# lingo-db/lingo-db

Hardware: AMD Instinct MI355X
Metric: tpch_sf100_geomean_ms (lower is better)
Workload: dtype int64/int128 decimal

## Files before the change

lingo-db_amd/csrc/ldb_core.hip:

```cpp
#include "ldb_internal.h"
#include "ldb_device.h"
#include "ldb_chain.h"
#include <algorithm>
#include <cstdlib>
#include <memory>

static thread_local char g_err[1024] = "";
void ldb_set_error(const char* fmt, ...) {
   va_list ap;
   va_start(ap, fmt);
   vsnprintf(g_err, sizeof(g_err), fmt, ap);
   va_end(ap);
}
extern "C" const char* ldb_gpu_last_error(void) { return g_err; }

#include <atomic>
#include <functional>
#include <mutex>
static std::mutex g_opt_mu;
static std::atomic<int64_t> g_option_epoch{0};
static std::unordered_map<std::string, int64_t> g_opts;
int64_t ldb_option(const char* name, int64_t dflt) {
   std::lock_guard<std::mutex> lock(g_opt_mu);
   auto it = g_opts.find(name);
   if (it != g_opts.end()) return it->second;
   std::string env = "LDB_";
   for (const char* c = name; *c; c++) env += (char) toupper((unsigned char) *c);
   int64_t v = dflt;
   if (const char* e = getenv(env.c_str())) v = atoll(e);
   g_opts[name] = v;
   return v;
}
extern "C" int32_t ldb_gpu_set_option(const char* name, int64_t value) {
   if (!name) LDB_FAIL(LDB_ERR_INVALID, "set_option: NULL name");
   static const char* known[] = {"jit", "jit_min_rows", "lazy_filter", "lazy_min_rows", "join_ordered", "join_chained", "gb_ordered", "gb_sorted", "zone_maps", "zone_min_rows", "gb_direct", "gb_wgs_per_cu", "gb_partition", "gb_partition_min_rows", "join_radix", "join_radix_min_rows", "join_radix_min_table_bytes", "join_radix_part_bytes", "probe_batch", "debug_check", "join_direct", "join_rank", "join_coarse", "dict_encode", "dict_min_rows", "comm_transport", "comm_timeout_ms", "desc_cache", "desc_cache_mb", "plan_replay", "scan_single_pass", "lazy_strings", "lazy_strings_min_rows", "gb_partition_wc", "join_radix_wc", "join_radix_lds", "gb_dense_out", "gb_partition_values", "join_pair32", "gb_dense_keys", "jit_async", "jit_threads", "jit_disk_cache", "join_all_match", "topk_short_select", "gb_fits64", "join_coarse_fine", "join_coarse_filtered", "compact_wide_tiles", "compact_max_words", "join_fuse_max_conjuncts", "join_coarse_finest", "jit_min_rows_like", "scan_split", "jit_share_compiles"};
   bool ok = false;
   for (const char* k : known) ok |= strcmp(k, name) == 0;
   if (!ok) LDB_FAIL(LDB_ERR_INVALID, "set_option: unknown option '%s'", name);
   std::lock_guard<std::mutex> lock(g_opt_mu);
   g_opts[name] = value;
   g_option_epoch.fetch_add(1);
   return LDB_OK;
}
extern "C" int64_t ldb_gpu_get_option(const char* name) {
   if (!name) return -1;
   std::lock_guard<std::mutex> lock(g_opt_mu);
   auto it = g_opts.find(name);
   if (it != g_opts.end()) return it->second;
   std::string env = "LDB_";
   for (const char* c = name; *c; c++) env += (char) toupper((unsigned char) *c);
   if (const char* e = getenv(env.c_str())) return atoll(e);
   return -1;
}

double ldb_host_trace_threshold() {
   static const double thr = [] {
      const char* e = getenv("LDB_HOST_TRACE");
      return e && *e ? atof(e) : -1.0;
   }();
   return thr;
}
static size_t ldb_size_class(size_t bytes) {
   if (bytes <= 256) return 256;
   const int lg = 63 - __builtin_clzll((unsigned long long) (bytes - 1));
   const size_t step = (size_t) 1 << (lg >= 3 ? lg - 3 : 0);
   return (bytes + step - 1) / step * step;
}
static void ldb_cache_release(ldb_ctx* ctx) {
   for (auto& kv : ctx->parked)
      for (void* p : kv.second) (void) hipFreeAsync(p, ctx->stream);
   ctx->parked.clear();
   ctx->cache_bytes = 0;
}
int32_t ldb_dev_alloc(ldb_ctx* ctx, void** out, size_t bytes) {
   const size_t cls = ctx->cache_on ? ldb_size_class(bytes + 16) : bytes + 16;
   if (ctx->cache_on) {
      auto it = ctx->parked.find(cls);
      if (it != ctx->parked.end() && !it->second.empty()) {
         std::pop_heap(it->second.begin(), it->second.end(), std::greater<void*>());
         *out = it->second.back();
         it->second.pop_back();
         ctx->cache_bytes -= cls;
         ctx->live[*out] = cls;
         return LDB_OK;
      }
   }
   hipError_t e;
   {
      LdbSlow slow_("hipMallocAsync", cls);
      e = hipMallocAsync(out, cls, ctx->stream);
   }
   if (e != hipSuccess && ctx->cache_bytes) {
      (void) hipGetLastError();
      ldb_cache_release(ctx);
      (void) hipStreamSynchronize(ctx->stream);
      e = hipMallocAsync(out, cls, ctx->stream);
   }
   LDB_HIP(e);
   if (ctx->cache_on) ctx->live[*out] = cls;
   return LDB_OK;
}
void ldb_dev_free(ldb_ctx* ctx, void* p) {
   if (!p) return;
   auto dref = ctx->desc_blocks.find(p);
   if (dref != ctx->desc_blocks.end()) {
      if (dref->second > 0) dref->second--;
      else {
         ctx->desc_underflows++;
         if (ldb_host_trace_threshold() >= 0) fprintf(stderr, "[ldb] descriptor %p given back twice\n", p);
      }
      return;
   }
   if (!ctx->shared.empty()) {
      auto sh = ctx->shared.find(p);
      if (sh != ctx->shared.end()) {
         if (--sh->second == 0) ctx->shared.erase(sh);
         return;
      }
// ... 2030 lines not shown
```

lingo-db_amd/csrc/ldb_join.hip:

```cpp
#include "ldb_internal.h"
#include "ldb_join_kernel.h"
#include "ldb_jit.h"
#include <cmath>
#include "ldb_chain.h"
#include <algorithm>
#include <memory>

struct ldb_hashtable {
   ldb_ctx* ctx = nullptr;
   ldb_rel* build = nullptr;
   std::vector<ldb_colref> keys;
   uint64_t* slots = nullptr;
   uint64_t cap = 0;
   int32_t key32 = 0;
   int32_t unique = 0;
   int32_t ordered_slots = 0;
   int64_t kmin = 0, kmax = -1;
   uint64_t kmult = 0;
   uint32_t kmult32 = 0, ksh = 0;
   int32_t slot32 = 0;
   uint32_t* key_bits = nullptr;
   int32_t chained = 0;
   uint32_t* next = nullptr;
   int32_t direct = 0;
// ... 12 lines not shown
   }
};

__global__ void k_join_build(const DJoin* __restrict__ d);
__global__ void k_join_key_range(const DJoin* __restrict__ d, long long* __restrict__ out);
__global__ void k_join_key_bits(const DJoin* __restrict__ d);
__global__ void k_join_rank_bits(const DJoin* __restrict__ d);
__global__ void k_join_rank_perm(const DJoin* __restrict__ d);
__global__ void k_rank_coarse(const uint64_t* __restrict__ tab, uint64_t n_words, uint32_t* __restrict__ coarse, uint32_t coarse_words, uint32_t shift) {
   for (uint32_t c = blockIdx.x * blockDim.x + threadIdx.x; c < coarse_words; c += gridDim.x * blockDim.x) {
      uint32_t m = 0;
      for (uint32_t b = 0; b < 32; b++) {
         const uint64_t bit = (uint64_t) c * 32 + b;
         uint32_t any;
         if (shift == 6) {
            const uint64_t w = bit * 2;
            any = (w < n_words ? (uint32_t) tab[w] : 0u) | (w + 1 < n_words ? (uint32_t) tab[w + 1] : 0u);
         } else if (shift == 5) {
            any = bit < n_words ? (uint32_t) tab[bit] : 0u;
         } else {
            const uint64_t w = bit >> (5u - shift);
            const uint32_t piece = (uint32_t) (bit & ((1u << (5u - shift)) - 1u)), width = 1u << shift;
            any = w < n_words ? ((uint32_t) tab[w] >> (piece * width)) & ((1u << width) - 1u) : 0u;
         }
         if (any) m |= 1u << b;
      }
      coarse[c] = m;
   }
}
__global__ __launch_bounds__(256) void k_rank_prefix_chain(uint64_t* __restrict__ tab, uint64_t n_words, uint64_t n_tiles, unsigned long long* __restrict__ total,
                                                           unsigned long long* __restrict__ status, unsigned long long* __restrict__ ticket, unsigned long long ticket_base,
                                                           unsigned long long epoch) {
   __shared__ unsigned long long s_tile;
   __shared__ uint32_t s_wave[4];
   __shared__ uint32_t s_prefix;
   if (threadIdx.x == 0) s_tile = atomicAdd(ticket, 1ull) - ticket_base;
   __syncthreads();
   const uint64_t tile = s_tile;
   const uint64_t base = tile * CHAIN_TILE + (uint64_t) threadIdx.x * CHAIN_ITEMS;
   uint32_t bits[CHAIN_ITEMS];
   uint32_t sum = 0;
#pragma unroll
   for (int k = 0; k < CHAIN_ITEMS; k++) {
      bits[k] = base + k < n_words ? (uint32_t) tab[base + k] : 0u;
      sum += (uint32_t) __popc(bits[k]);
   }
   uint32_t agg;
   uint32_t excl = d_block_scan256<uint32_t>(sum, s_wave, &agg);
   if (threadIdx.x < 64) {
      const uint32_t prefix = d_chain_prefix<uint32_t, 32>(status, tile, epoch, agg, threadIdx.x);
      if (threadIdx.x == 0) s_prefix = prefix;
   }
   __syncthreads();
   excl += s_prefix;
   if (total && tile == n_tiles - 1 && threadIdx.x == 0) *total = (unsigned long long) s_prefix + agg;
#pragma unroll
   for (int k = 0; k < CHAIN_ITEMS; k++) {
      if (base + k < n_words) tab[base + k] = (uint64_t) bits[k] | ((uint64_t) excl << 32);
      excl += (uint32_t) __popc(bits[k]);
   }
}
__global__ void k_join_probe_pairs(const DJoin* __restrict__ d);
__global__ void k_join_probe_pairs_count(const DJoin* __restrict__ d);
__global__ void k_join_probe_count(const DJoin* __restrict__ d);
__global__ void k_join_probe_exists(const DJoin* __restrict__ d);
__global__ void k_join_probe_unique(const DJoin* __restrict__ d);
__global__ void k_join_probe_markbuild(const DJoin* __restrict__ d);
__global__ void k_join_flags_bitmap(const uint8_t* __restrict__ flags, uint64_t n, int anti, uint64_t* __restrict__ bitmap, unsigned long long* __restrict__ counter) {
   join_flags_bitmap_body(flags, n, anti, bitmap, counter);
}
__global__ void k_join_flags_bitmap2(const uint8_t* __restrict__ flags, const uint8_t* __restrict__ not_flags, uint64_t n, uint64_t* __restrict__ bitmap, unsigned long long* __restrict__ counter) {
   join_flags_bitmap_body(flags, n, 0, bitmap, counter, not_flags);
}

static const char* JOIN_SPEC_SRC =
   "extern \"C\" __global__ void k_join_build_spec(const DJoin* __restrict__ d) { join_build_body(LDB_META, d); }\n"
   "extern \"C\" __global__ void k_join_probe_pairs_spec(const DJoin* __restrict__ d) { join_probe_pairs_body(LDB_META, d); }\n"
   "extern \"C\" __global__ void k_join_probe_pairs_count_spec(const DJoin* __restrict__ d) { join_probe_pairs_count_body(LDB_META, d); }\n"
   "extern \"C\" __global__ void k_join_probe_count_spec(const DJoin* __restrict__ d) { join_probe_count_body(LDB_META, d); }\n"
   "extern \"C\" __global__ void k_join_probe_exists_spec(const DJoin* __restrict__ d) { join_probe_exists_body(LDB_META, d); }\n"
   "extern \"C\" __global__ void k_join_probe_unique_spec(const DJoin* __restrict__ d) { join_probe_unique_body(LDB_META, d); }\n"
   "extern \"C\" __global__ void k_join_probe_markbuild_spec(const DJoin* __restrict__ d) { join_probe_markbuild_body(LDB_META, d); }\n";

typedef void (*join_kernel_t)(const DJoin*);
static int32_t launch_join(ldb_ctx* ctx, const DJoin* h, const DJoin* d, int grid, const char* prof_name, const char* spec_name, join_kernel_t generic) {
   hipFunction_t spec = nullptr;
   if (ldb_jit_wanted((int64_t) h->n_rows)) {
      auto meta = std::make_unique<DJoin>();
      memcpy(meta.get(), h, sizeof(DJoin));
      meta->n_rows = meta->cap = meta->slots = meta->out_probe = meta->out_build = meta->out_cap = 0;
      meta->counter = meta->bitmap = meta->mark = meta->mark2 = meta->match = meta->flags = 0;
      meta->kmin = meta->kmax = 0;
      meta->kmult = 0;
      meta->kmult32 = meta->ksh = 0;
      meta->key_bits = 0;
      meta->next = 0;
      meta->coarse = 0;
      meta->coarse_words = 0;
      ldb_jit_strip_keys(meta->bkeys);
      ldb_jit_strip_keys(meta->pkeys);
      for (int p = 0; p < LDB_MAX_PREDS; p++) ldb_jit_strip_pred(meta->ppreds[p]);
      for (int p = 0; p < LDB_MAX_M2PREDS; p++) ldb_jit_strip_pred(meta->m2preds[p]);
      for (int k = 0; k < LDB_MAX_RESID; k++) {
         ldb_jit_strip_col(meta->resid[k].pcol);
         ldb_jit_strip_col(meta->resid[k].bcol);
      }
      std::string why;
      std::string one;
      for (const char* line = JOIN_SPEC_SRC; *line;) {
         const char* nl = strchr(line, '\n');
         const size_t len = nl ? (size_t) (nl - line) + 1 : strlen(line);
         std::string l(line, len);
         if (l.find(std::string(" ") + spec_name + "(") != std::string::npos) one = l;
         line += len;
      }
      spec = ldb_jit_kernel(ctx->device, "ldb_join_kernel.h", "DJoin", one.empty() ? JOIN_SPEC_SRC : one.c_str(), spec_name, meta.get(), sizeof(DJoin), &why);
   }
   const unsigned lds = h->has_coarse ? 4u * h->coarse_words : 0u;
   const bool big_lds = lds > 40u * 1024u;
   const bool tiles = h->n_ppreds > 0;
   const unsigned block = (h->has_coarse && !tiles) ? (big_lds ? 1024u : 512u) : 256u;
   if (h->has_coarse && !tiles) grid = (int) std::max<int64_t>(1, std::min<int64_t>(((int64_t) h->n_rows + block - 1) / block, (int64_t) ctx->cus * (big_lds ? 1 : 4)));
   if (big_lds) {
      if (spec) (void) hipFuncSetAttribute((const void*) spec, hipFuncAttributeMaxDynamicSharedMemorySize, (int) lds);
      else (void) hipFuncSetAttribute((const void*) generic, hipFuncAttributeMaxDynamicSharedMemorySize, (int) lds);
      (void) hipGetLastError();
   }
   LdbProf prof_(ctx, prof_name);
   if (spec) {
      void* params[] = {(void*) &d};
      LDB_HIP(hipModuleLaunchKernel(spec, (unsigned) grid, 1, 1, block, 1, 1, lds, ctx->stream, params, nullptr));
   } else {
      hipLaunchKernelGGL(generic, dim3(grid), dim3(block), lds, ctx->stream, d);
   }
   LDB_HIP(hipGetLastError());
   return LDB_OK;
}

bool ldb_join_jit_check(std::string* log) {
   auto m = std::make_unique<DJoin>();
   memset(m.get(), 0, sizeof(DJoin));
   m->key32 = 1;
   m->kind = LDB_JOIN_INNER;
   m->has_bitmap = 1;
   m->ordered_slots = 1;
   m->has_key_bits = 1;
   m->build_unique = 1;
   m->slot32 = 1;
   m->bkeys.n_keys = m->pkeys.n_keys = 1;
   m->bkeys.cols[0].type = m->pkeys.cols[0].type = LDB_T_INT32;
   m->bkeys.cols[0].width = m->pkeys.cols[0].width = 4;
   m->n_ppreds = 2;
   for (int p = 0; p < 2; p++) {
      m->ppreds[p].col.type = LDB_T_DATE32;
      m->ppreds[p].col.width = 4;
      m->ppreds[p].op = p ? LDB_F_LTE : LDB_F_GTE;
      m->ppreds[p].lo = p ? 9861 : 9131;
      m->ppreds[p].same_col = p;
   }
   if (const char* shape = getenv("LDB_JIT_CHECK_SHAPE")) {
      if (!strcmp(shape, "fk_count")) {
         m->n_ppreds = 0;
         m->has_key_bits = 0;
         m->has_bitmap = 0;
      }
   }
   if (!ldb_jit_compile_only("ldb_join_kernel.h", "DJoin", JOIN_SPEC_SRC, m.get(), sizeof(DJoin), log)) return false;
   m->n_ppreds = 0;
   m->ordered_slots = 0;
   m->slot32 = 0;
   m->has_key_bits = 0;
   m->direct = 1;
   if (!ldb_jit_compile_only("ldb_join_kernel.h", "DJoin", JOIN_SPEC_SRC, m.get(), sizeof(DJoin), log)) return false;
   m->direct = 2;
   m->rank_sorted = 1;
   if (!ldb_jit_compile_only("ldb_join_kernel.h", "DJoin", JOIN_SPEC_SRC, m.get(), sizeof(DJoin), log)) return false;
   m->rank_sorted = 0;
   m->kind = LDB_JOIN_SEMI;
   if (!ldb_jit_compile_only("ldb_join_kernel.h", "DJoin", JOIN_SPEC_SRC, m.get(), sizeof(DJoin), log)) return false;
   m->rank_sorted = 1;
   m->has_coarse = 32 | 6;
   return ldb_jit_compile_only("ldb_join_kernel.h", "DJoin", JOIN_SPEC_SRC, m.get(), sizeof(DJoin), log);
}

__global__ void k_word_pop(const uint64_t* __restrict__ bitmap, uint32_t* __restrict__ pop, uint64_t n_words) {
   for (uint64_t w = blockIdx.x * (uint64_t) blockDim.x + threadIdx.x; w < n_words; w += (uint64_t) gridDim.x * blockDim.x) pop[w] = (uint32_t) __popcll(bitmap[w]);
}
__global__ void k_bitmap_expand(const uint64_t* __restrict__ bitmap, const uint32_t* __restrict__ word_off, uint32_t* __restrict__ out, uint64_t n_words) {
   const uint32_t lane = threadIdx.x & 63;
   const uint64_t wave = (blockIdx.x * (uint64_t) blockDim.x + threadIdx.x) >> 6;
   const uint64_t n_waves = ((uint64_t) gridDim.x * blockDim.x) >> 6;
   for (uint64_t w = wave; w < n_words; w += n_waves) {
      uint64_t m = bitmap[w];
      if ((m >> lane) & 1) out[word_off[w] + d_rank_in(m)] = (uint32_t) (w * 64 + lane);
   }
}
__global__ void k_bitmap_expand_sparse(const uint64_t* __restrict__ bitmap, const uint32_t* __restrict__ word_off, uint32_t* __restrict__ out, uint64_t n_words) {
   for (uint64_t w = blockIdx.x * (uint64_t) blockDim.x + threadIdx.x; w < n_words; w += (uint64_t) gridDim.x * blockDim.x) {
      uint64_t m = bitmap[w];
      if (!m) continue;
      uint32_t at = word_off[w];
      const uint32_t base = (uint32_t) (w * 64);
      while (m) {
         out[at++] = base + (uint32_t) __builtin_ctzll(m);
         m &= m - 1;
// ... 330 lines not shown
   ht->unique = build_unique;
   auto hp = std::make_unique<DJoin>();
   DJoin* h = hp.get();
   memset(h, 0, sizeof(*h));
   LDB_TRY(ldb_make_dkeys(build, keys, n_keys, &h->bkeys));
   const DCol& k0 = h->bkeys.cols[0];
   ht->key32 = (n_keys == 1 && (k0.type == LDB_T_INT32 || k0.type == LDB_T_DATE32 || k0.type == LDB_T_CHAR4 || k0.type == LDB_T_INT16 || k0.type == LDB_T_INT8)) ? 1 : 0;
   ht->cap = std::max<uint64_t>(64, next_pow2_u64((uint64_t) build->n_rows * 2));
   h->n_rows = (uint64_t) build->n_rows;
   h->key32 = ht->key32;
   uint32_t* dflags;
   LDB_TRY(ldb_counters(ctx, 1, (uint64_t**) &dflags));
   h->flags = (uint64_t) dflags;
   h->has_flags = 1;
   const bool ordered_enabled = ldb_option("join_ordered", 1) != 0;
   if (ht->key32 && ordered_enabled && build->n_rows > 0) {
      long long got[2];
      const ldb_table* kt = build->sides[(size_t) keys[0].side].table;
      int64_t clo = 0, chi = -1;
      if (!kt->cols[(size_t) keys[0].col].validity && ldb_column_range(ctx, kt, keys[0].col, &clo, &chi) == LDB_OK && clo <= chi) {
         got[0] = clo;
         got[1] = chi;
      } else {
         long long* range = (long long*) (ctx->d_scratch + 32);
         const long long init[2] = {INT64_MAX, INT64_MIN};
         LDB_TRY(ldb_h2d_small(ctx, range, init, 16));
         LdbDesc<DJoin> dr_desc(ctx);
         LDB_TRY(dr_desc.upload(h, sizeof(*h)));
         DJoin* dr = dr_desc.p;
         hipLaunchKernelGGL(k_join_key_range, dim3(ldb_grid_for(ctx, build->n_rows, 256, 8)), dim3(256), 0, ctx->stream, dr, range);
         LDB_TRY(LDB_READBACK(ctx, got, range, 16));
         dr_desc.release();
      }
      const unsigned __int128 range0 = got[0] <= got[1] ? (unsigned __int128) ((__int128) got[1] - got[0]) + 1 : 0;
      bool ranked = false;
      if (range0 > 0 && build_unique && ldb_option("join_direct", 1) != 0 && ldb_option("join_rank", 1) != 0 && range0 <= ((unsigned __int128) 1 << 32) &&
          (range0 <= (unsigned __int128) std::max<int64_t>(4096, 64 * build->n_rows) || range0 <= ((unsigned __int128) 1 << 26)) && got[0] >= INT32_MIN && got[1] <= INT32_MAX && build->n_rows < (int64_t) LDB_NULL_ROW) {
         const uint64_t n_words = (uint64_t) (range0 / 32) + 1;
         uint64_t* tab = nullptr;
         LDB_TRY(ldb_dev_alloc(ctx, (void**) &tab, 8 * (size_t) n_words));
         ht->slots = tab;
         LDB_HIP(hipMemsetAsync(tab, 0, 8 * (size_t) n_words, ctx->stream));
         unsigned long long* counter;
         LDB_TRY(ldb_counters(ctx, 3, (uint64_t**) &counter));
         uint64_t* d_total = (uint64_t*) (counter + 2);
         h->direct = 2;
         h->kmin = got[0];
         h->kmax = got[1];
         h->slots = (uint64_t) tab;
         h->counter = (uint64_t) counter;
         LdbDesc<DJoin> dr_desc(ctx);
         LDB_TRY(dr_desc.upload(h, sizeof(*h)));
         DJoin* dr = dr_desc.p;
         {
            LdbProf prof_(ctx, "k_join_build");
            hipLaunchKernelGGL(k_join_rank_bits, dim3(ldb_grid_for(ctx, build->n_rows, 256, 8)), dim3(256), 0, ctx->stream, dr);
            const uint64_t n_tiles = (n_words + CHAIN_TILE - 1) / CHAIN_TILE;
            ChainCall c;
            LDB_TRY(ldb_chain_begin(ctx, n_tiles, false, &c));
            hipLaunchKernelGGL(k_rank_prefix_chain, dim3((unsigned) n_tiles), dim3(256), 0, ctx->stream, tab, n_words, n_tiles, (unsigned long long*) d_total, c.status, c.ticket, c.ticket_base, c.epoch);
            if (hipGetLastError() != hipSuccess) return ldb_chain_failed(ctx);
         }
         uint64_t back[3] = {0, 0, 0};
         uint32_t fl[2] = {0, 0};
         LDB_TRY(LDB_READBACK(ctx, back, counter, 24));
         LDB_TRY(LDB_READBACK(ctx, fl, dflags, 8));
         if (back[0] == back[2]) {
            ranked = true;
            ht->direct = 2;
            ht->kmin = got[0];
            ht->kmax = got[1];
            ht->cap = (uint64_t) range0;
            ht->slot_bytes = 8 * (size_t) n_words;
            ht->rank_sorted = (fl[0] & 4u) ? 0 : 1;
            uint32_t shift = 6;
            uint64_t cwords = (uint64_t) (range0 / 64 / 32) + 1;
            const double density = range0 > 0 ? (double) back[2] / (double) range0 : 1.0;
            const double pass64 = 1.0 - pow(1.0 - density, 64.0), pass16 = 1.0 - pow(1.0 - density, 16.0);
            const bool coarse_on = ldb_option("join_coarse", 1) != 0;
            bool want = coarse_on && cwords * 4 <= 40 * 1024 && (unsigned __int128) back[2] * 64 * 2 <= range0;
            if (coarse_on && ldb_option("join_coarse_fine", 1) != 0 && pass16 <= 0.7) {
               const uint64_t fine_words = (uint64_t) (range0 / 16 / 32) + 1;
               const bool small = fine_words * 4 <= 40 * 1024;
               if (small || (fine_words * 4 <= 156 * 1024 && (!want || pass64 > 0.25))) {
                  shift = 4;
                  cwords = fine_words;
                  want = true;
               }
            }
            if (coarse_on && ldb_option("join_coarse_finest", 1) != 0 && want && shift == 4 && cwords * 4 <= 16 * 1024) {
               while (shift > 0 && ((uint64_t) (range0 >> (shift - 1)) / 32 + 1) * 4 <= 16 * 1024 && 1.0 - pow(1.0 - density, (double) (1u << shift)) > 0.1) shift--;
               cwords = (uint64_t) (range0 >> shift) / 32 + 1;
            }
            if (want) {
               LDB_TRY(ldb_dev_alloc(ctx, (void**) &ht->coarse, 4 * (size_t) cwords));
               ht->coarse_words = (uint32_t) cwords;
               ht->coarse_shift = shift;
               hipLaunchKernelGGL(k_rank_coarse, dim3((unsigned) ((cwords + 255) / 256)), dim3(256), 0, ctx->stream, (const uint64_t*) tab, n_words, ht->coarse, (uint32_t) cwords, shift);
               LDB_HIP(hipGetLastError());
            }
            if (!ht->rank_sorted) {
               LDB_TRY(ldb_dev_alloc(ctx, (void**) &ht->next, 4 * (size_t) (build->n_rows ? build->n_rows : 1)));
               h->next = (uint64_t) ht->next;
               LdbDesc<DJoin> dp_desc(ctx);
               LDB_TRY(dp_desc.upload(h, sizeof(*h)));
               DJoin* dp = dp_desc.p;
               hipLaunchKernelGGL(k_join_rank_perm, dim3(ldb_grid_for(ctx, build->n_rows, 256, 8)), dim3(256), 0, ctx->stream, dp);
               LDB_HIP(hipGetLastError());
               dp_desc.release();
            }
         } else {
            ldb_dev_free(ctx, tab);
            ht->slots = nullptr;
            h->direct = 0;
            h->slots = 0;
            h->counter = 0;
            ht->unique = 0;
            build_unique = 0;
         }
         dr_desc.release();
         LDB_TRY(ldb_counters(ctx, 1, (uint64_t**) &dflags));
         h->flags = (uint64_t) dflags;
      }
      if (ranked) {
         *out = ht.release();
         return LDB_OK;
      }
      if (range0 > 0 && ldb_option("join_direct", 1) != 0 && range0 <= (unsigned __int128) std::max<int64_t>(1024, 8 * build->n_rows) && range0 < ((unsigned __int128) 1 << 31) &&
          got[0] >= INT32_MIN && got[1] <= INT32_MAX) {
         ht->direct = 1;
         ht->kmin = got[0];
         ht->kmax = got[1];
         ht->cap = (uint64_t) range0;
         if (range0 <= ((unsigned __int128) 1 << 27) && range0 >= 4096) {
            const size_t words = (size_t) ((range0 + 31) / 32);
            LDB_TRY(ldb_dev_alloc(ctx, (void**) &ht->key_bits, 4 * words));
            LDB_HIP(hipMemsetAsync(ht->key_bits, 0, 4 * words, ctx->stream));
         }
      } else if (got[0] <= got[1]) {
         ht->ordered_slots = 1;
         ht->kmin = got[0];
         ht->kmax = got[1];
         ht->kmult = (uint64_t) ((((unsigned __int128) ht->cap) << 32) / ((unsigned __int128) (got[1] - got[0]) + 1));
         {
            const unsigned __int128 range128 = (unsigned __int128) ((__int128) got[1] - got[0]) + 1;
            if (ht->cap <= (1ull << 31) && range128 <= ((unsigned __int128) 1 << 32) && got[0] >= INT32_MIN && got[1] <= INT32_MAX) {
               uint64_t range = (uint64_t) range128;
               uint32_t ksh = 0;
               while ((range << ksh) < ht->cap) ksh++;
               const unsigned __int128 km = (((unsigned __int128) ht->cap) << 32) / (unsigned __int128) (range << ksh);
               ht->kmult32 = km > 0xFFFFFFFFull ? 0xFFFFFFFFu : (uint32_t) km;
               ht->ksh = ksh;
               ht->slot32 = 1;
            }
         }
         const unsigned __int128 range = (unsigned __int128) ((__int128) got[1] - got[0]) + 1;
         if (range <= ((unsigned __int128) 1 << 27)) {
            const size_t words = (size_t) ((range + 31) / 32);
            LDB_TRY(ldb_dev_alloc(ctx, (void**) &ht->key_bits, 4 * words));
            LDB_HIP(hipMemsetAsync(ht->key_bits, 0, 4 * words, ctx->stream));
         }
      }
   }
   const bool force_chained = ldb_option("join_chained", 0) == 1;
   if (force_chained && !ht->direct) {
      ht->ordered_slots = 0;
      ldb_dev_free(ctx, ht->key_bits);
// ... 557 lines not shown
```

lingo-db_amd/csrc/ldb_join_kernel.h:

```cpp
#pragma once
#include "ldb_keys.h"

#define LDB_MAX_RESID 2
#define LDB_MAX_M2PREDS 2
struct DJoinResid {
   DCol pcol;
   DCol bcol;
   int32_t op;
   int32_t pad;
};
struct DJoin {
   uint64_t n_rows;
   uint64_t cap;
   uint64_t slots;
   uint64_t out_probe;
   uint64_t out_build;
   uint64_t out_cap;
   uint64_t counter;
   uint64_t bitmap;
   uint64_t mark;
   uint64_t mark2;
   uint64_t match;
   uint64_t flags;
   int64_t kmin, kmax;
// ... 697 lines not shown
   const uint32_t lane = threadIdx.x & 63;
   const uint64_t wave = d_wave_id();
   const uint64_t n_waves = ((uint64_t) gridDim.x * blockDim.x) >> 6;
   const uint32_t* chunk_off = gptr<uint32_t>(d->match);
   uint32_t* out_probe = gptr_mut<uint32_t>(d->out_probe);
   uint32_t* out_build = gptr_mut<uint32_t>(d->out_build);
   const uint64_t out_cap = d->out_cap;
   for (uint64_t w0 = wave * JP_U; w0 < n_chunks; w0 += n_waves * JP_U) {
      uint64_t rows[JP_U], at[JP_U];
      bool act[JP_U];
      uint32_t c[JP_U], emitted[JP_U];
#pragma unroll
      for (int u = 0; u < JP_U; u++) {
         rows[u] = (w0 + u) * 64 + lane;
         act[u] = rows[u] < n;
      }
      d_pairs_of_rows<JP_U>(m, d, rows, act, c);
#pragma unroll
      for (int u = 0; u < JP_U; u++) {
         uint32_t incl = c[u];
         for (int off = 1; off < 64; off <<= 1) {
            uint32_t up = __shfl_up(incl, off);
            if (lane >= (uint32_t) off) incl += up;
         }
         at[u] = (uint64_t) (w0 + u < n_chunks ? chunk_off[w0 + u] : 0u) + (incl - c[u]);
         emitted[u] = 0;
         act[u] = act[u] && c[u] != 0;
      }
      uint32_t again[JP_U];
      d_probe_batch<JP_U>(m, d, rows, act, again, [&](int u, uint32_t brow) {
         if (at[u] + emitted[u] < out_cap) {
            out_probe[at[u] + emitted[u]] = (uint32_t) rows[u];
            out_build[at[u] + emitted[u]] = brow;
         }
         emitted[u]++;
         return m.kind != LDB_JOIN_SINGLE;
      });
#pragma unroll
      for (int u = 0; u < JP_U; u++) {
         if (act[u] && emitted[u] == 0 && at[u] < out_cap) {
            out_probe[at[u]] = (uint32_t) rows[u];
            out_build[at[u]] = LDB_NULL_ROW;
         }
      }
   }
}

__device__ __forceinline__ void join_probe_count_body(const DJoin& m, const DJoin* __restrict__ d) {
   const uint64_t n = d->n_rows;
   d_stage_coarse(m, d);
   unsigned long long local = 0;
   const uint32_t lane = threadIdx.x & 63;
   const uint64_t wave = d_wave_id();
   const uint64_t n_waves = ((uint64_t) gridDim.x * blockDim.x) >> 6;
   const uint64_t n_tiles = (n + 64 * JOIN_BATCH - 1) / (64 * JOIN_BATCH);
   DProbePipe<JOIN_BATCH> pipe;
   pipe.start(m, d, wave * JOIN_BATCH * 64, n_waves * JOIN_BATCH * 64, n);
   auto tile = [&](uint64_t t, auto par) __attribute__((always_inline)) {
      uint64_t rows[JOIN_BATCH];
      bool act[JOIN_BATCH];
      uint32_t mt[JOIN_BATCH];
#pragma unroll
      for (int u = 0; u < JOIN_BATCH; u++) {
         rows[u] = (t * JOIN_BATCH + u) * 64 + lane;
         act[u] = rows[u] < n;
      }
      pipe.step(m, d, t * JOIN_BATCH * 64, n, par);
      d_eval_conj_batch<JOIN_BATCH>(m.ppreds, d->ppreds, m.n_ppreds, rows, act);
      d_probe_batch<JOIN_BATCH>(m, d, rows, act, mt, [](int, uint32_t) { return true; }, pipe.keys(m), pipe.words(m));
#pragma unroll
      for (int u = 0; u < JOIN_BATCH; u++) local += mt[u];
   };
   d_tile_loop<JOIN_BATCH>(m, wave, n_tiles, n_waves, tile);
   for (int off = 32; off > 0; off >>= 1) local += __shfl_down(local, off);
   if (lane == 0 && local) atomicAdd(gptr_mut<unsigned long long>(d->counter) + 1, local);
}

#define JT_BLOCK 256
#define JT_U 8
#define JT_ROWS (JT_BLOCK * JT_U)
#ifndef JT_PB
#define JT_PB 4
#endif
struct JoinTile {
   unsigned short q[JT_ROWS];
   unsigned long long bm[JT_ROWS / 64];
   uint32_t qn;
};
__device__ __forceinline__ void d_tile_filter(const DJoin& m, const DJoin* __restrict__ d, uint64_t base, uint64_t n, JoinTile& st) {
   const uint32_t t = threadIdx.x, lane = t & 63;
   if (t < JT_ROWS / 64) st.bm[t] = 0;
   if (t == 0) st.qn = 0;
   __syncthreads();
   uint64_t rows[JT_U];
   bool pass[JT_U];
#pragma unroll
   for (int u = 0; u < JT_U; u++) {
      rows[u] = base + (uint64_t) u * JT_BLOCK + t;
      pass[u] = rows[u] < n;
   }
   d_eval_conj_batch<JT_U>(m.ppreds, d->ppreds, m.n_ppreds, rows, pass);
#pragma unroll
   for (int u = 0; u < JT_U; u++) {
      const uint64_t mask = __ballot(pass[u]);
      uint32_t b = 0;
      if (mask != 0 && lane == (uint32_t) __builtin_ctzll(mask)) b = atomicAdd(&st.qn, (uint32_t) __popcll(mask));
      b = __shfl(b, mask ? __builtin_ctzll(mask) : 0);
      if (pass[u]) st.q[b + (uint32_t) __popcll(mask & ((1ull << lane) - 1ull))] = (unsigned short) (u * JT_BLOCK + t);
   }
   __syncthreads();
}
template <typename ON_MATCH, typename AFTER>
__device__ __forceinline__ void d_tile_probe(const DJoin& m, const DJoin* __restrict__ d, uint64_t base, JoinTile& st, ON_MATCH on_match, AFTER after) {
#ifdef JT_EXTRA_SYNC
   __syncthreads();
#endif
   const uint32_t qn = st.qn;
   for (uint32_t j0 = 0; j0 < qn; j0 += JT_PB * JT_BLOCK) {
      uint64_t rows[JT_PB];
      uint32_t rel[JT_PB], mt[JT_PB];
      bool act[JT_PB];
#pragma unroll
      for (int u = 0; u < JT_PB; u++) {
         const uint32_t j = j0 + (uint32_t) u * JT_BLOCK + threadIdx.x;
         act[u] = j < qn;
         rel[u] = act[u] ? st.q[j] : 0u;
         rows[u] = base + rel[u];
      }
      d_probe_batch<JT_PB>(m, d, rows, act, mt, [&](int u, uint32_t b) { return on_match(rel[u], b); });
#pragma unroll
      for (int u = 0; u < JT_PB; u++)
         if (act[u]) after(rel[u], mt[u]);
   }
}
template <typename AFTER>
__device__ __forceinline__ void d_tile_probe_first(const DJoin& m, const DJoin* __restrict__ d, uint64_t base, JoinTile& st, AFTER after) {
   const uint32_t qn = st.qn;
   for (uint32_t j0 = 0; j0 < qn; j0 += JT_PB * JT_BLOCK) {
      uint64_t rows[JT_PB];
      uint32_t rel[JT_PB], brow[JT_PB];
      bool act[JT_PB];
#pragma unroll
      for (int u = 0; u < JT_PB; u++) {
         const uint32_t j = j0 + (uint32_t) u * JT_BLOCK + threadIdx.x;
         act[u] = j < qn;
         rel[u] = act[u] ? st.q[j] : 0u;
         rows[u] = base + rel[u];
      }
      d_probe_first<JT_PB>(m, d, rows, act, brow);
#ifdef JOIN_DEBUG_COUNTS
      {
         unsigned long long* dc = gptr_mut<unsigned long long>(d->counter);
         unsigned long long q = 0, hit = 0, inr = 0;
#pragma unroll
         for (int u = 0; u < JT_PB; u++) {
            q += act[u] ? 1 : 0;
            hit += (act[u] && brow[u] != LDB_NULL_ROW) ? 1 : 0;
            if (act[u]) {
               const CV c = KV(m.pkeys, d->pkeys).col(0);
               const int64_t kv = d_load_i64(c, (uint32_t) rows[u]);
               if (kv >= d->kmin && kv <= d->kmax) {
                  const uint64_t r = (uint64_t) (kv - d->kmin);
                  inr += (gptr<uint32_t>(d->key_bits)[r >> 5] >> (r & 31)) & 1u;
               }
            }
         }
         atomicAdd(dc + 2, q);
         atomicAdd(dc + 3, inr);
         atomicAdd(dc + 4, hit);
      }
#endif
#pragma unroll
      for (int u = 0; u < JT_PB; u++)
         if (act[u]) after(rel[u], brow[u]);
   }
}
__device__ __forceinline__ void d_tile_flush(const DJoin* __restrict__ d, uint64_t tile, uint64_t n_words, JoinTile& st, unsigned long long& local) {
   uint64_t* bitmap = gptr_mut<uint64_t>(d->bitmap);
   __syncthreads();
   if (threadIdx.x < JT_ROWS / 64) {
      const uint64_t w = tile * (JT_ROWS / 64) + threadIdx.x;
      if (w < n_words) {
         bitmap[w] = st.bm[threadIdx.x];
         local += (unsigned long long) __popcll(st.bm[threadIdx.x]);
      }
   }
   __syncthreads();
}
__device__ __forceinline__ void d_block_count_add(const DJoin* __restrict__ d, unsigned long long local) {
   if (threadIdx.x < 64) {
      for (int off = 32; off > 0; off >>= 1) local += __shfl_down(local, off);
      if (threadIdx.x == 0 && local) atomicAdd(gptr_mut<unsigned long long>(d->counter), local);
   }
}

__device__ __forceinline__ void join_probe_unique_filtered_body(const DJoin& m, const DJoin* __restrict__ d) {
   __shared__ JoinTile st;
   const uint64_t n = d->n_rows;
   const uint64_t n_words = (n + 63) / 64, n_tiles = (n + JT_ROWS - 1) / JT_ROWS;
   uint32_t* match = gptr_mut<uint32_t>(d->match);
   unsigned long long local = 0;
   for (uint64_t tile = blockIdx.x; tile < n_tiles; tile += gridDim.x) {
      const uint64_t base = tile * JT_ROWS;
      d_tile_filter(m, d, base, n, st);
      d_tile_probe_first(m, d, base, st, [&](uint32_t r, uint32_t b) {
         if (b != LDB_NULL_ROW) {
            match[base + r] = b;
            atomicOr(&st.bm[r >> 6], 1ull << (r & 63));
         }
      });
      d_tile_flush(d, tile, n_words, st, local);
   }
   d_block_count_add(d, local);
}

#define JE_U 4
__device__ __forceinline__ void join_probe_exists_body(const DJoin& m, const DJoin* __restrict__ d) {
   const uint64_t n = d->n_rows;
   d_stage_coarse(m, d);
   if (m.n_ppreds > 0) {
      __shared__ JoinTile st;
      const uint64_t n_words = (n + 63) / 64, n_tiles = (n + JT_ROWS - 1) / JT_ROWS;
      unsigned long long local = 0;
      for (uint64_t tile = blockIdx.x; tile < n_tiles; tile += gridDim.x) {
         const uint64_t base = tile * JT_ROWS;
         d_tile_filter(m, d, base, n, st);
         d_tile_probe_first(m, d, base, st, [&](uint32_t r, uint32_t b) {
            if (m.kind == LDB_JOIN_ANTI ? b == LDB_NULL_ROW : b != LDB_NULL_ROW) atomicOr(&st.bm[r >> 6], 1ull << (r & 63));
         });
         d_tile_flush(d, tile, n_words, st, local);
      }
      d_block_count_add(d, local);
      return;
   }
   const uint64_t n_words = (n + 63) / 64;
   const uint32_t lane = threadIdx.x & 63;
   const uint64_t wave = d_wave_id();
   const uint64_t n_waves = ((uint64_t) gridDim.x * blockDim.x) >> 6;
   uint64_t* bitmap = gptr_mut<uint64_t>(d->bitmap);
   uint8_t* mark = gptr_mut<uint8_t>(d->mark);
   unsigned long long local = 0;
   DProbePipe<JE_U> pipe;
   pipe.start(m, d, wave * JE_U * 64, n_waves * JE_U * 64, n);
   auto tile = [&](uint64_t w0, auto par) __attribute__((always_inline)) {
      uint64_t rows[JE_U];
      bool act[JE_U];
      uint32_t first[JE_U];
#pragma unroll
      for (int u = 0; u < JE_U; u++) {
         rows[u] = (w0 + u) * 64 + lane;
         act[u] = rows[u] < n;
      }
      pipe.step(m, d, w0 * 64, n, par);
      d_probe_first<JE_U>(m, d, rows, act, first, pipe.keys(m), pipe.words(m));
#pragma unroll
      for (int u = 0; u < JE_U; u++) {
         const bool hit = first[u] != LDB_NULL_ROW;
         const bool keep = act[u] && (m.kind == LDB_JOIN_ANTI ? !hit : hit);
         if (m.has_mark && act[u]) mark[rows[u]] = hit ? 1 : 0;
         const uint64_t mm = __ballot(keep);
         if (lane == 0 && w0 + u < n_words) {
            bitmap[w0 + u] = mm;
            local += (unsigned long long) __popcll(mm);
         }
      }
   };
   d_tile_loop<JE_U>(m, wave * JE_U, n_words, n_waves * JE_U, tile);
   if (lane == 0 && local) atomicAdd(gptr_mut<unsigned long long>(d->counter), local);
}

__device__ __forceinline__ void join_probe_markbuild_body(const DJoin& m, const DJoin* __restrict__ d) {
   const uint64_t n = d->n_rows;
   d_stage_coarse(m, d);
   uint8_t* flags = gptr_mut<uint8_t>(d->mark);
   if (m.n_ppreds > 0) {
      __shared__ JoinTile st;
      const uint64_t n_tiles = (n + JT_ROWS - 1) / JT_ROWS;
      for (uint64_t tile = blockIdx.x; tile < n_tiles; tile += gridDim.x) {
         const uint64_t base = tile * JT_ROWS;
         d_tile_filter(m, d, base, n, st);
         d_tile_probe(
            m, d, base, st,
            [&](uint32_t, uint32_t b) {
               flags[b] = 1;
               return true;
            },
            [](uint32_t, uint32_t) {});
         __syncthreads();
      }
      return;
   }
   const uint32_t lane = threadIdx.x & 63;
   const uint64_t wave = d_wave_id();
   const uint64_t n_waves = ((uint64_t) gridDim.x * blockDim.x) >> 6;
   const uint64_t n_tiles = (n + 64 * JE_U - 1) / (64 * JE_U);
   DProbePipe<JE_U> pipe;
   pipe.start(m, d, wave * JE_U * 64, n_waves * JE_U * 64, n);
   auto tile = [&](uint64_t t, auto par) __attribute__((always_inline)) {
      uint64_t rows[JE_U];
      bool act[JE_U];
      uint32_t mt[JE_U];
#pragma unroll
      for (int u = 0; u < JE_U; u++) {
         rows[u] = (t * JE_U + u) * 64 + lane;
         act[u] = rows[u] < n;
      }
      pipe.step(m, d, t * JE_U * 64, n, par);
      d_probe_batch<JE_U>(
         m, d, rows, act, mt,
         [&](int u, uint32_t b) {
            flags[b] = 1;
            if (m.n_m2preds > 0) {
               bool also = true;
               LDB_UNROLL
               for (int p = 0; p < m.n_m2preds; p++)
                  if (also) also = d_eval_pred(PV(m.m2preds[p], d->m2preds[p]), rows[u]);
               if (also) gptr_mut<uint8_t>(d->mark2)[b] = 1;
            }
            return true;
         },
         pipe.keys(m), pipe.words(m));
   };
   d_tile_loop<JE_U>(m, wave, n_tiles, n_waves, tile);
}
__device__ __forceinline__ void join_flags_bitmap_body(const uint8_t* __restrict__ flags, uint64_t n, int anti, uint64_t* __restrict__ bitmap,
                                                       unsigned long long* __restrict__ counter, const uint8_t* __restrict__ not_flags = nullptr) {
   const uint64_t n_words = (n + 63) / 64;
   const uint32_t lane = threadIdx.x & 63;
   const uint64_t wave = d_wave_id();
   const uint64_t n_waves = ((uint64_t) gridDim.x * blockDim.x) >> 6;
   unsigned long long local = 0;
   for (uint64_t w = wave; w < n_words; w += n_waves) {
      const uint64_t i = w * 64 + lane;
      bool keep = i < n && ((flags[i] != 0) != (anti != 0));
      if (not_flags && keep) keep = not_flags[i] == 0;
      uint64_t mm = __ballot(keep);
      if (lane == 0) {
         bitmap[w] = mm;
         local += (unsigned long long) __popcll(mm);
      }
   }
   if (lane == 0 && local) atomicAdd(counter, local);
}

__device__ __forceinline__ void join_probe_unique_body(const DJoin& m, const DJoin* __restrict__ d) {
   d_stage_coarse(m, d);
   if (m.n_ppreds > 0 && m.has_bitmap) {
      join_probe_unique_filtered_body(m, d);
      return;
   }
   const uint64_t n = d->n_rows;
   const uint64_t n_words = (n + 63) / 64;
   const uint32_t lane = threadIdx.x & 63;
   const uint64_t wave = d_wave_id();
   const uint64_t n_waves = ((uint64_t) gridDim.x * blockDim.x) >> 6;
   uint64_t* bitmap = gptr_mut<uint64_t>(d->bitmap);
   uint32_t* match = gptr_mut<uint32_t>(d->match);
   unsigned long long local = 0;
   DProbePipe<JE_U> pipe;
   pipe.start(m, d, wave * JE_U * 64, n_waves * JE_U * 64, n);
   auto tile = [&](uint64_t w0, auto par) __attribute__((always_inline)) {
      uint32_t brow[JE_U];
      uint64_t rows[JE_U];
      bool act[JE_U], pass[JE_U];
#pragma unroll
      for (int u = 0; u < JE_U; u++) {
         rows[u] = (w0 + u) * 64 + lane;
         act[u] = pass[u] = rows[u] < n;
      }
      pipe.step(m, d, w0 * 64, n, par);
      d_eval_conj_batch<JE_U>(m.ppreds, d->ppreds, m.n_ppreds, rows, pass);
// ... 15 lines not shown
```

Before: 3.611.

## Batch filtered join probes across multi-tile chunks with a ring queue

Filtered join probe kernels (exists, markbuild, unique-with-bitmap) now process chunks of several tiles per workgroup. Filter survivors accumulate in an LDS ring queue and are probed only in full batches, so lanes are not left idle when each tile passes few rows. The launch grid for these kernels is capped by row count, with a new join_tile_grid option to cap it further. The fine coarse-filter LDS limit is now derived from the remaining LDS beside the larger chunk struct. The cost is more static LDS per workgroup, which may lower occupancy, plus fewer workgroups on small inputs.

```diff
diff --git a/lingo-db_amd/csrc/ldb_core.hip b/lingo-db_amd/csrc/ldb_core.hip
--- a/lingo-db_amd/csrc/ldb_core.hip
+++ b/lingo-db_amd/csrc/ldb_core.hip
@@ -33,7 +33,7 @@
 }
 extern "C" int32_t ldb_gpu_set_option(const char* name, int64_t value) {
    if (!name) LDB_FAIL(LDB_ERR_INVALID, "set_option: NULL name");
-   static const char* known[] = {"jit", "jit_min_rows", "lazy_filter", "lazy_min_rows", "join_ordered", "join_chained", "gb_ordered", "gb_sorted", "zone_maps", "zone_min_rows", "gb_direct", "gb_wgs_per_cu", "gb_partition", "gb_partition_min_rows", "join_radix", "join_radix_min_rows", "join_radix_min_table_bytes", "join_radix_part_bytes", "probe_batch", "debug_check", "join_direct", "join_rank", "join_coarse", "dict_encode", "dict_min_rows", "comm_transport", "comm_timeout_ms", "desc_cache", "desc_cache_mb", "plan_replay", "scan_single_pass", "lazy_strings", "lazy_strings_min_rows", "gb_partition_wc", "join_radix_wc", "join_radix_lds", "gb_dense_out", "gb_partition_values", "join_pair32", "gb_dense_keys", "jit_async", "jit_threads", "jit_disk_cache", "join_all_match", "topk_short_select", "gb_fits64", "join_coarse_fine", "join_coarse_filtered", "compact_wide_tiles", "compact_max_words", "join_fuse_max_conjuncts", "join_coarse_finest", "jit_min_rows_like", "scan_split", "jit_share_compiles"};
+   static const char* known[] = {"jit", "jit_min_rows", "lazy_filter", "lazy_min_rows", "join_ordered", "join_chained", "gb_ordered", "gb_sorted", "zone_maps", "zone_min_rows", "gb_direct", "gb_wgs_per_cu", "gb_partition", "gb_partition_min_rows", "join_radix", "join_radix_min_rows", "join_radix_min_table_bytes", "join_radix_part_bytes", "probe_batch", "debug_check", "join_direct", "join_rank", "join_coarse", "dict_encode", "dict_min_rows", "comm_transport", "comm_timeout_ms", "desc_cache", "desc_cache_mb", "plan_replay", "scan_single_pass", "lazy_strings", "lazy_strings_min_rows", "gb_partition_wc", "join_radix_wc", "join_radix_lds", "gb_dense_out", "gb_partition_values", "join_pair32", "gb_dense_keys", "jit_async", "jit_threads", "jit_disk_cache", "join_all_match", "topk_short_select", "gb_fits64", "join_coarse_fine", "join_coarse_filtered", "compact_wide_tiles", "compact_max_words", "join_fuse_max_conjuncts", "join_coarse_finest", "jit_min_rows_like", "scan_split", "jit_share_compiles", "join_tile_grid"};
    bool ok = false;
    for (const char* k : known) ok |= strcmp(k, name) == 0;
    if (!ok) LDB_FAIL(LDB_ERR_INVALID, "set_option: unknown option '%s'", name);
diff --git a/lingo-db_amd/csrc/ldb_join.hip b/lingo-db_amd/csrc/ldb_join.hip
--- a/lingo-db_amd/csrc/ldb_join.hip
+++ b/lingo-db_amd/csrc/ldb_join.hip
@@ -118,6 +118,8 @@
    "extern \"C\" __global__ void k_join_probe_unique_spec(const DJoin* __restrict__ d) { join_probe_unique_body(LDB_META, d); }\n"
    "extern \"C\" __global__ void k_join_probe_markbuild_spec(const DJoin* __restrict__ d) { join_probe_markbuild_body(LDB_META, d); }\n";
 
+static constexpr uint64_t JOIN_FINE_LDS_MAX = 160 * 1024 - ((JT_STATIC_LDS + 15) & ~(size_t) 15);
+static_assert(JOIN_FINE_LDS_MAX >= 156250, "the fine filter of a 20 M key range (156 250 B) must still fit beside the chunk queue: fewer sub-tiles per chunk");
 typedef void (*join_kernel_t)(const DJoin*);
 static int32_t launch_join(ldb_ctx* ctx, const DJoin* h, const DJoin* d, int grid, const char* prof_name, const char* spec_name, join_kernel_t generic) {
    hipFunction_t spec = nullptr;
@@ -157,6 +159,12 @@
    const bool tiles = h->n_ppreds > 0;
    const unsigned block = (h->has_coarse && !tiles) ? (big_lds ? 1024u : 512u) : 256u;
    if (h->has_coarse && !tiles) grid = (int) std::max<int64_t>(1, std::min<int64_t>(((int64_t) h->n_rows + block - 1) / block, (int64_t) ctx->cus * (big_lds ? 1 : 4)));
+   const bool chunks = tiles && (generic == k_join_probe_exists || generic == k_join_probe_markbuild || (generic == k_join_probe_unique && h->has_bitmap));
+   if (chunks) {
+      grid = (int) std::max<int64_t>(1, std::min<int64_t>(grid, ((int64_t) h->n_rows + 2047) / 2048));
+      const int64_t cap = ldb_option("join_tile_grid", 0);
+      if (cap > 0) grid = (int) std::min<int64_t>(grid, cap);
+   }
    if (big_lds) {
       if (spec) (void) hipFuncSetAttribute((const void*) spec, hipFuncAttributeMaxDynamicSharedMemorySize, (int) lds);
       else (void) hipFuncSetAttribute((const void*) generic, hipFuncAttributeMaxDynamicSharedMemorySize, (int) lds);
@@ -653,7 +661,7 @@
             if (coarse_on && ldb_option("join_coarse_fine", 1) != 0 && pass16 <= 0.7) {
                const uint64_t fine_words = (uint64_t) (range0 / 16 / 32) + 1;
                const bool small = fine_words * 4 <= 40 * 1024;
-               if (small || (fine_words * 4 <= 156 * 1024 && (!want || pass64 > 0.25))) {
+               if (small || (fine_words * 4 <= JOIN_FINE_LDS_MAX && (!want || pass64 > 0.25))) {
                   shift = 4;
                   cwords = fine_words;
                   want = true;
diff --git a/lingo-db_amd/csrc/ldb_join_kernel.h b/lingo-db_amd/csrc/ldb_join_kernel.h
--- a/lingo-db_amd/csrc/ldb_join_kernel.h
+++ b/lingo-db_amd/csrc/ldb_join_kernel.h
@@ -803,16 +803,35 @@
 #ifndef JT_PB
 #define JT_PB 4
 #endif
-struct JoinTile {
-   unsigned short q[JT_ROWS];
-   unsigned long long bm[JT_ROWS / 64];
-   uint32_t qn;
+#ifndef JT_CHUNK_TILES
+#define JT_CHUNK_TILES 5
+#endif
+#define JT_BATCH (JT_PB * JT_BLOCK)
+#define JT_QCAP (JT_ROWS + JT_BATCH)
+static_assert(JT_CHUNK_TILES >= 1 && JT_CHUNK_TILES * JT_ROWS <= 65536, "a chunk-relative row number must fit the queue's unsigned short");
+template <int BM_WORDS>
+struct JoinChunk {
+   unsigned short q[JT_QCAP];
+   unsigned long long bm[BM_WORDS];
+   uint32_t qtail;
 };
-__device__ __forceinline__ void d_tile_filter(const DJoin& m, const DJoin* __restrict__ d, uint64_t base, uint64_t n, JoinTile& st) {
+typedef JoinChunk<JT_CHUNK_TILES * JT_ROWS / 64> JoinChunkBm;
+#define JT_STATIC_LDS sizeof(JoinChunkBm)
+typedef JoinChunk<1> JoinChunkNoBm;
+__device__ __forceinline__ uint32_t d_chunk_tiles(uint64_t n_tiles) {
+   const uint64_t per_wg = n_tiles / gridDim.x > 1 ? n_tiles / gridDim.x : 1;
+   const uint64_t trips = (per_wg + JT_CHUNK_TILES - 1) / JT_CHUNK_TILES;
+   return (uint32_t) ((per_wg + trips - 1) / trips);
+}
+template <int BM_WORDS>
+__device__ __forceinline__ void d_chunk_init(JoinChunk<BM_WORDS>& st) {
+   for (uint32_t w = threadIdx.x; w < (uint32_t) BM_WORDS; w += JT_BLOCK) st.bm[w] = 0;
+   if (threadIdx.x == 0) st.qtail = 0;
+   __syncthreads();
+}
+template <int BM_WORDS>
+__device__ __forceinline__ void d_chunk_filter(const DJoin& m, const DJoin* __restrict__ d, uint64_t base, uint32_t rel0, uint64_t n, JoinChunk<BM_WORDS>& st) {
    const uint32_t t = threadIdx.x, lane = t & 63;
-   if (t < JT_ROWS / 64) st.bm[t] = 0;
-   if (t == 0) st.qn = 0;
-   __syncthreads();
    uint64_t rows[JT_U];
    bool pass[JT_U];
 #pragma unroll
@@ -825,112 +844,121 @@
    for (int u = 0; u < JT_U; u++) {
       const uint64_t mask = __ballot(pass[u]);
       uint32_t b = 0;
-      if (mask != 0 && lane == (uint32_t) __builtin_ctzll(mask)) b = atomicAdd(&st.qn, (uint32_t) __popcll(mask));
+      if (mask != 0 && lane == (uint32_t) __builtin_ctzll(mask)) b = atomicAdd(&st.qtail, (uint32_t) __popcll(mask));
       b = __shfl(b, mask ? __builtin_ctzll(mask) : 0);
-      if (pass[u]) st.q[b + (uint32_t) __popcll(mask & ((1ull << lane) - 1ull))] = (unsigned short) (u * JT_BLOCK + t);
+      if (pass[u]) st.q[(b + (uint32_t) __popcll(mask & ((1ull << lane) - 1ull))) % JT_QCAP] = (unsigned short) (rel0 + (uint32_t) u * JT_BLOCK + t);
    }
    __syncthreads();
 }
-template <typename ON_MATCH, typename AFTER>
-__device__ __forceinline__ void d_tile_probe(const DJoin& m, const DJoin* __restrict__ d, uint64_t base, JoinTile& st, ON_MATCH on_match, AFTER after) {
-#ifdef JT_EXTRA_SYNC
-   __syncthreads();
+template <int BM_WORDS, typename ON_MATCH>
+__device__ __forceinline__ void d_chunk_probe(const DJoin& m, const DJoin* __restrict__ d, uint64_t cbase, JoinChunk<BM_WORDS>& st, uint32_t head, uint32_t cnt, ON_MATCH on_match) {
+   uint64_t rows[JT_PB];
+   uint32_t rel[JT_PB], mt[JT_PB];
+   bool act[JT_PB];
+#pragma unroll
+   for (int u = 0; u < JT_PB; u++) {
+      const uint32_t o = (uint32_t) u * JT_BLOCK + threadIdx.x;
+      act[u] = o < cnt;
+      rel[u] = act[u] ? st.q[(head + o) % JT_QCAP] : 0u;
+      rows[u] = cbase + rel[u];
+   }
+   d_probe_batch<JT_PB>(m, d, rows, act, mt, [&](int u, uint32_t b) { return on_match(rel[u], b); });
+}
+template <int BM_WORDS, typename AFTER>
+__device__ __forceinline__ void d_chunk_probe_first(const DJoin& m, const DJoin* __restrict__ d, uint64_t cbase, JoinChunk<BM_WORDS>& st, uint32_t head, uint32_t cnt, AFTER after) {
+   uint64_t rows[JT_PB];
+   uint32_t rel[JT_PB], brow[JT_PB];
+   bool act[JT_PB];
+#pragma unroll
+   for (int u = 0; u < JT_PB; u++) {
+      const uint32_t o = (uint32_t) u * JT_BLOCK + threadIdx.x;
+      act[u] = o < cnt;
+      rel[u] = act[u] ? st.q[(head + o) % JT_QCAP] : 0u;
+      rows[u] = cbase + rel[u];
+   }
+   d_probe_first<JT_PB>(m, d, rows, act, brow);
+#ifdef JOIN_DEBUG_COUNTS
+   {
+      unsigned long long* dc = gptr_mut<unsigned long long>(d->counter);
+      unsigned long long q = 0, hit = 0, inr = 0;
+#pragma unroll
+      for (int u = 0; u < JT_PB; u++) {
+         q += act[u] ? 1 : 0;
+         hit += (act[u] && brow[u] != LDB_NULL_ROW) ? 1 : 0;
+         if (act[u]) {
+            const CV c = KV(m.pkeys, d->pkeys).col(0);
+            const int64_t kv = d_load_i64(c, (uint32_t) rows[u]);
+            if (kv >= d->kmin && kv <= d->kmax) {
+               const uint64_t r = (uint64_t) (kv - d->kmin);
+               inr += (gptr<uint32_t>(d->key_bits)[r >> 5] >> (r & 31)) & 1u;
+            }
+         }
+      }
+      atomicAdd(dc + 2, q);
+      atomicAdd(dc + 3, inr);
+      atomicAdd(dc + 4, hit);
+   }
 #endif
-   const uint32_t qn = st.qn;
-   for (uint32_t j0 = 0; j0 < qn; j0 += JT_PB * JT_BLOCK) {
-      uint64_t rows[JT_PB];
-      uint32_t rel[JT_PB], mt[JT_PB];
-      bool act[JT_PB];
-#pragma unroll
-      for (int u = 0; u < JT_PB; u++) {
-         const uint32_t j = j0 + (uint32_t) u * JT_BLOCK + threadIdx.x;
-         act[u] = j < qn;
-         rel[u] = act[u] ? st.q[j] : 0u;
-         rows[u] = base + rel[u];
-      }
-      d_probe_batch<JT_PB>(m, d, rows, act, mt, [&](int u, uint32_t b) { return on_match(rel[u], b); });
-#pragma unroll
-      for (int u = 0; u < JT_PB; u++)
-         if (act[u]) after(rel[u], mt[u]);
-   }
-}
-template <typename AFTER>
-__device__ __forceinline__ void d_tile_probe_first(const DJoin& m, const DJoin* __restrict__ d, uint64_t base, JoinTile& st, AFTER after) {
-   const uint32_t qn = st.qn;
-   for (uint32_t j0 = 0; j0 < qn; j0 += JT_PB * JT_BLOCK) {
-      uint64_t rows[JT_PB];
-      uint32_t rel[JT_PB], brow[JT_PB];
-      bool act[JT_PB];
-#pragma unroll
-      for (int u = 0; u < JT_PB; u++) {
-         const uint32_t j = j0 + (uint32_t) u * JT_BLOCK + threadIdx.x;
-         act[u] = j < qn;
-         rel[u] = act[u] ? st.q[j] : 0u;
-         rows[u] = base + rel[u];
-      }
-      d_probe_first<JT_PB>(m, d, rows, act, brow);
-#ifdef JOIN_DEBUG_COUNTS
-      {
-         unsigned long long* dc = gptr_mut<unsigned long long>(d->counter);
-         unsigned long long q = 0, hit = 0, inr = 0;
-#pragma unroll
-         for (int u = 0; u < JT_PB; u++) {
-            q += act[u] ? 1 : 0;
-            hit += (act[u] && brow[u] != LDB_NULL_ROW) ? 1 : 0;
-            if (act[u]) {
-               const CV c = KV(m.pkeys, d->pkeys).col(0);
-               const int64_t kv = d_load_i64(c, (uint32_t) rows[u]);
-               if (kv >= d->kmin && kv <= d->kmax) {
-                  const uint64_t r = (uint64_t) (kv - d->kmin);
-                  inr += (gptr<uint32_t>(d->key_bits)[r >> 5] >> (r & 31)) & 1u;
-               }
-            }
-         }
-         atomicAdd(dc + 2, q);
-         atomicAdd(dc + 3, inr);
-         atomicAdd(dc + 4, hit);
-      }
-#endif
-#pragma unroll
-      for (int u = 0; u < JT_PB; u++)
-         if (act[u]) after(rel[u], brow[u]);
-   }
-}
-__device__ __forceinline__ void d_tile_flush(const DJoin* __restrict__ d, uint64_t tile, uint64_t n_words, JoinTile& st, unsigned long long& local) {
+#pragma unroll
+   for (int u = 0; u < JT_PB; u++)
+      if (act[u]) after(rel[u], brow[u]);
+}
+template <int BM_WORDS, typename BATCH>
+__device__ __forceinline__ void d_chunk_run(const DJoin& m, const DJoin* __restrict__ d, uint64_t cbase, uint32_t tiles, uint64_t n, JoinChunk<BM_WORDS>& st, BATCH batch) {
+   uint32_t head = 0, tail = 0;
+   for (uint32_t s = 0; s < tiles; s++) {
+      d_chunk_filter(m, d, cbase + (uint64_t) s * JT_ROWS, s * JT_ROWS, n, st);
+      tail = (uint32_t) __builtin_amdgcn_readfirstlane((int) st.qtail);
+      for (; tail - head >= JT_BATCH; head += JT_BATCH) batch(head, (uint32_t) JT_BATCH);
+      __syncthreads();
+   }
+   if (tail != head) batch(head, tail - head);
+}
+__device__ __forceinline__ void d_chunk_flush(const DJoin* __restrict__ d, uint64_t cbase, uint32_t tiles, uint64_t n_words, JoinChunkBm& st, unsigned long long& local) {
    uint64_t* bitmap = gptr_mut<uint64_t>(d->bitmap);
    __syncthreads();
-   if (threadIdx.x < JT_ROWS / 64) {
-      const uint64_t w = tile * (JT_ROWS / 64) + threadIdx.x;
-      if (w < n_words) {
-         bitmap[w] = st.bm[threadIdx.x];
-         local += (unsigned long long) __popcll(st.bm[threadIdx.x]);
-      }
-   }
+   for (uint32_t w = threadIdx.x; w < tiles * (JT_ROWS / 64); w += JT_BLOCK) {
+      const uint64_t gw = cbase / 64 + w;
+      if (gw < n_words) {
+         const unsigned long long v = st.bm[w];
+         bitmap[gw] = v;
+         local += (unsigned long long) __popcll(v);
+      }
+      st.bm[w] = 0;
+   }
+   if (threadIdx.x == 0) st.qtail = 0;
    __syncthreads();
 }
+__device__ __forceinline__ void d_chunk_reset(JoinChunkNoBm& st) {
+   if (threadIdx.x == 0) st.qtail = 0;
+   __syncthreads();
+}
 __device__ __forceinline__ void d_block_count_add(const DJoin* __restrict__ d, unsigned long long local) {
-   if (threadIdx.x < 64) {
-      for (int off = 32; off > 0; off >>= 1) local += __shfl_down(local, off);
-      if (threadIdx.x == 0 && local) atomicAdd(gptr_mut<unsigned long long>(d->counter), local);
-   }
+   for (int off = 32; off > 0; off >>= 1) local += __shfl_down(local, off);
+   if ((threadIdx.x & 63) == 0 && local) atomicAdd(gptr_mut<unsigned long long>(d->counter), local);
 }
 
 __device__ __forceinline__ void join_probe_unique_filtered_body(const DJoin& m, const DJoin* __restrict__ d) {
-   __shared__ JoinTile st;
+   __shared__ JoinChunkBm st;
    const uint64_t n = d->n_rows;
    const uint64_t n_words = (n + 63) / 64, n_tiles = (n + JT_ROWS - 1) / JT_ROWS;
+   const uint32_t ct = d_chunk_tiles(n_tiles);
+   const uint64_t n_chunks = (n_tiles + ct - 1) / ct;
    uint32_t* match = gptr_mut<uint32_t>(d->match);
    unsigned long long local = 0;
-   for (uint64_t tile = blockIdx.x; tile < n_tiles; tile += gridDim.x) {
-      const uint64_t base = tile * JT_ROWS;
-      d_tile_filter(m, d, base, n, st);
-      d_tile_probe_first(m, d, base, st, [&](uint32_t r, uint32_t b) {
-         if (b != LDB_NULL_ROW) {
-            match[base + r] = b;
-            atomicOr(&st.bm[r >> 6], 1ull << (r & 63));
-         }
+   d_chunk_init(st);
+   for (uint64_t chunk = blockIdx.x; chunk < n_chunks; chunk += gridDim.x) {
+      const uint64_t cbase = chunk * ct * JT_ROWS;
+      const uint32_t tiles = (uint32_t) (n_tiles - chunk * ct < ct ? n_tiles - chunk * ct : ct);
+      d_chunk_run(m, d, cbase, tiles, n, st, [&](uint32_t head, uint32_t cnt) {
+         d_chunk_probe_first(m, d, cbase, st, head, cnt, [&](uint32_t r, uint32_t b) {
+            if (b != LDB_NULL_ROW) {
+               match[cbase + r] = b;
+               atomicOr(&st.bm[r >> 6], 1ull << (r & 63));
+            }
+         });
       });
-      d_tile_flush(d, tile, n_words, st, local);
+      d_chunk_flush(d, cbase, tiles, n_words, st, local);
    }
    d_block_count_add(d, local);
 }
@@ -940,16 +968,21 @@
    const uint64_t n = d->n_rows;
    d_stage_coarse(m, d);
    if (m.n_ppreds > 0) {
-      __shared__ JoinTile st;
+      __shared__ JoinChunkBm st;
       const uint64_t n_words = (n + 63) / 64, n_tiles = (n + JT_ROWS - 1) / JT_ROWS;
+      const uint32_t ct = d_chunk_tiles(n_tiles);
+      const uint64_t n_chunks = (n_tiles + ct - 1) / ct;
       unsigned long long local = 0;
-      for (uint64_t tile = blockIdx.x; tile < n_tiles; tile += gridDim.x) {
-         const uint64_t base = tile * JT_ROWS;
-         d_tile_filter(m, d, base, n, st);
-         d_tile_probe_first(m, d, base, st, [&](uint32_t r, uint32_t b) {
-            if (m.kind == LDB_JOIN_ANTI ? b == LDB_NULL_ROW : b != LDB_NULL_ROW) atomicOr(&st.bm[r >> 6], 1ull << (r & 63));
+      d_chunk_init(st);
+      for (uint64_t chunk = blockIdx.x; chunk < n_chunks; chunk += gridDim.x) {
+         const uint64_t cbase = chunk * ct * JT_ROWS;
+         const uint32_t tiles = (uint32_t) (n_tiles - chunk * ct < ct ? n_tiles - chunk * ct : ct);
+         d_chunk_run(m, d, cbase, tiles, n, st, [&](uint32_t head, uint32_t cnt) {
+            d_chunk_probe_first(m, d, cbase, st, head, cnt, [&](uint32_t r, uint32_t b) {
+               if (m.kind == LDB_JOIN_ANTI ? b == LDB_NULL_ROW : b != LDB_NULL_ROW) atomicOr(&st.bm[r >> 6], 1ull << (r & 63));
+            });
          });
-         d_tile_flush(d, tile, n_words, st, local);
+         d_chunk_flush(d, cbase, tiles, n_words, st, local);
       }
       d_block_count_add(d, local);
       return;
@@ -995,19 +1028,21 @@
    d_stage_coarse(m, d);
    uint8_t* flags = gptr_mut<uint8_t>(d->mark);
    if (m.n_ppreds > 0) {
-      __shared__ JoinTile st;
+      __shared__ JoinChunkNoBm st;
       const uint64_t n_tiles = (n + JT_ROWS - 1) / JT_ROWS;
-      for (uint64_t tile = blockIdx.x; tile < n_tiles; tile += gridDim.x) {
-         const uint64_t base = tile * JT_ROWS;
-         d_tile_filter(m, d, base, n, st);
-         d_tile_probe(
-            m, d, base, st,
-            [&](uint32_t, uint32_t b) {
+      const uint32_t ct = d_chunk_tiles(n_tiles);
+      const uint64_t n_chunks = (n_tiles + ct - 1) / ct;
+      d_chunk_init(st);
+      for (uint64_t chunk = blockIdx.x; chunk < n_chunks; chunk += gridDim.x) {
+         const uint64_t cbase = chunk * ct * JT_ROWS;
+         const uint32_t tiles = (uint32_t) (n_tiles - chunk * ct < ct ? n_tiles - chunk * ct : ct);
+         d_chunk_run(m, d, cbase, tiles, n, st, [&](uint32_t head, uint32_t cnt) {
+            d_chunk_probe(m, d, cbase, st, head, cnt, [&](uint32_t, uint32_t b) {
                flags[b] = 1;
                return true;
-            },
-            [](uint32_t, uint32_t) {});
-         __syncthreads();
+            });
+         });
+         d_chunk_reset(st);
       }
       return;
    }
```

Result: slower. 4.163 (+15.3%).
